# omid-arhami/topolow

Hardware: AMD Instinct MI355X
Metric: relaxation iterations/sec (NxN pairs) (higher is better)
Workload: dtype f32

## Files before the change

topolow_amd/csrc/relax_kernels.h:

```cpp
#pragma once

#include <hip/hip_runtime.h>
#include <type_traits>
#include "relax_common.h"

namespace topolow {

constexpr int kThreads = 256;
constexpr int kWaves = kThreads / 64;

template <int THREADS_, int RPW_, int CHUNK_, int PRIO_ = 0, int MINWAVES_ = 1>
struct StageCfg {
  static constexpr int MINWAVES = MINWAVES_;
  static constexpr int PRIO = PRIO_;
  static constexpr int THREADS = THREADS_;
  static constexpr int WAVES = THREADS_ / 64;
  static constexpr int RPW = RPW_;
  static constexpr int ROWS = WAVES * RPW_;
  static constexpr int CHUNK = CHUNK_;
};

template <typename real> struct Math;
template <> struct Math<float> {
  static __device__ __forceinline__ float sqrt(float x) { return __builtin_amdgcn_sqrtf(x); }
  static __device__ __forceinline__ float rcp(float x) { return __builtin_amdgcn_rcpf(x); }
  static constexpr float far() { return kFarF32; }
};
template <> struct Math<double> {
#ifdef TOPOLOW_F64_IEEE
  static __device__ __forceinline__ double sqrt(double x) { return ::sqrt(x); }
  static __device__ __forceinline__ double rcp(double x) { return 1.0 / x; }
#else
  static __device__ __forceinline__ double sqrt(double x) {
    const double y0 = __builtin_amdgcn_rsq(x);
    double g = x * y0, h = 0.5 * y0;
    const double e1 = fma(-h, g, 0.5);
    g = fma(g, e1, g);
    h = fma(h, e1, h);
    g = fma(fma(-g, g, x), h, g);
    return x > 0.0 ? g : 0.0;
  }
  static __device__ __forceinline__ double rcp(double x) {
    double y = __builtin_amdgcn_rcp(x);
    y = fma(fma(-x, y, 1.0), y, y);
    return fma(fma(-x, y, 1.0), y, y);
  }
#endif
  static constexpr double far() { return kFarF64; }
};

__device__ __forceinline__ float uniform(float v) {
  return __builtin_bit_cast(float, __builtin_amdgcn_readfirstlane(__builtin_bit_cast(int, v)));
}
__device__ __forceinline__ double uniform(double v) {
  const long long b = __builtin_bit_cast(long long, v);
  const int lo = __builtin_amdgcn_readfirstlane((int)(b & 0xffffffffll));
  const int hi = __builtin_amdgcn_readfirstlane((int)(b >> 32));
  return __builtin_bit_cast(double, ((long long)hi << 32) | (unsigned int)lo);
}

template <typename real>
__device__ __forceinline__ real wave_sum(real v) {
#pragma unroll
  for (int m = 32; m >= 1; m >>= 1) v += __shfl_xor(v, m, 64);
  return v;
}

__device__ __forceinline__ float wave_sum_dpp(float v) {
  auto dpp = [](float x, auto ctrl, auto row_mask) {
    return __builtin_bit_cast(float, __builtin_amdgcn_update_dpp(0, __builtin_bit_cast(int, x), decltype(ctrl)::value,
                                                                 decltype(row_mask)::value, 0xf, true));
  };
  using std::integral_constant;
  v += dpp(v, integral_constant<int, 0xB1>{}, integral_constant<int, 0xf>{});
  v += dpp(v, integral_constant<int, 0x4E>{}, integral_constant<int, 0xf>{});
  v += dpp(v, integral_constant<int, 0x141>{}, integral_constant<int, 0xf>{});
  v += dpp(v, integral_constant<int, 0x140>{}, integral_constant<int, 0xf>{});
  v += dpp(v, integral_constant<int, 0x142>{}, integral_constant<int, 0xa>{});
  v += dpp(v, integral_constant<int, 0x143>{}, integral_constant<int, 0xc>{});
  return __builtin_bit_cast(float, __builtin_amdgcn_readlane(__builtin_bit_cast(int, v), 63));
}

typedef __amdgpu_buffer_rsrc_t row_rsrc_t;
__device__ __forceinline__ row_rsrc_t make_row_rsrc(const uint32_t* block, int row_in_block, int ld) {
  const uint32_t* row = block + enc_index(row_in_block, 0, ld);
  return __builtin_amdgcn_make_buffer_rsrc(const_cast<uint32_t*>(row),  0,
                                           enc_row_span_bytes(row_in_block, ld), 0x00020000);
}
__device__ __forceinline__ uint4 load_words(row_rsrc_t rsrc, int byte_off) {
  typedef unsigned int u32x4 __attribute__((ext_vector_type(4)));
  const u32x4 v = __builtin_amdgcn_raw_buffer_load_b128(rsrc, byte_off, 0, 0);
  return make_uint4(v.x, v.y, v.z, v.w);
}

template <int DIM, typename real, int THREADS, int CHUNK>
__device__ __forceinline__ void stage_points(const real* __restrict__ pos, int cb, int cw,
                                             real* lds_pos, int tid) {
  constexpr int kMaxVec = (CHUNK * DIM * (int)sizeof(real) / 16 + THREADS - 1) / THREADS;
  const uint4* src = reinterpret_cast<const uint4*>(pos + (size_t)cb * DIM);
  uint4* dst = reinterpret_cast<uint4*>(lds_pos);
  const int nvec = cw * DIM * (int)sizeof(real) / 16;
  uint4 tmp[kMaxVec];
#pragma unroll
  for (int v = 0; v < kMaxVec; ++v) {
    const int q = tid + v * THREADS;
    tmp[v] = src[q < nvec ? q : 0];
  }
#pragma unroll
  for (int v = 0; v < kMaxVec; ++v) {
    const int q = tid + v * THREADS;
    if (q < nvec) dst[q] = tmp[v];
  }
}

template <int DIM, typename real>
__device__ __forceinline__ void load_points(const real* lds_pos, int c4, real (&pc)[4][DIM]) {
  constexpr int kPer16 = 16 / (int)sizeof(real);
  constexpr int kVec = 4 * DIM / kPer16;
  const uint4* src = reinterpret_cast<const uint4*>(lds_pos + (size_t)c4 * DIM);
#pragma unroll
  for (int v = 0; v < kVec; ++v) {
    const uint4 u = src[v];
    if constexpr (sizeof(real) == 4) {
      pc[(4 * v + 0) / DIM][(4 * v + 0) % DIM] = __builtin_bit_cast(float, u.x);
      pc[(4 * v + 1) / DIM][(4 * v + 1) % DIM] = __builtin_bit_cast(float, u.y);
      pc[(4 * v + 2) / DIM][(4 * v + 2) % DIM] = __builtin_bit_cast(float, u.z);
      pc[(4 * v + 3) / DIM][(4 * v + 3) % DIM] = __builtin_bit_cast(float, u.w);
    } else {
      pc[(2 * v + 0) / DIM][(2 * v + 0) % DIM] =
          __builtin_bit_cast(double, ((unsigned long long)u.y << 32) | u.x);
      pc[(2 * v + 1) / DIM][(2 * v + 1) % DIM] =
          __builtin_bit_cast(double, ((unsigned long long)u.w << 32) | u.z);
    }
  }
}

template <int DIM, typename real, bool THR, bool ERR = false, bool CNT = false>
__device__ __forceinline__ void pair_accum(const real (&pc)[DIM], const real (&pi)[DIM],
                                           uint32_t w, real ks, real cg, real (&acc)[DIM],
                                           float* err = nullptr, unsigned* cnt_wave = nullptr) {
  real dx[DIM];
  real s = 0;
#pragma unroll
  for (int d = 0; d < DIM; ++d) {
    dx[d] = pc[d] - pi[d];
    s = fma(dx[d], dx[d], s);
  }
  const real r = Math<real>::sqrt(s);
  const real inv = Math<real>::rcp(r + (real)0.01);
  const real t = (real)bits_f32(THR ? (w & ~kCodeMask) : w);
  bool spring;
  if constexpr (THR) {
    const uint32_t code = w & kCodeMask;
    spring = (code == 0u) | ((code == 1u) & (r < t)) | ((code == 2u) & (r > t));
  } else {
// ... 528 lines not shown
              pair_error_rows2<DIM, false>(pc[3], pi2, w4[t][0].w, w4[t][1].w, err, cnt_wave);
            }
          }
        }
        if (lane == 0) cnt += cnt_wave;
        err_d += (double)err;
        err = 0.0f;
        continue;
      }
    }
#pragma unroll
    for (int t = 0; t < kGroups; ++t) {
      const int c4 = lane * 4 + t * 256;
      if (c4 >= cw) continue;
      const int col = cb + c4;
      real pc[4][DIM];
      load_points<DIM, real>(lds_pos, c4, pc);
#pragma unroll
      for (int r = 0; r < RPW; ++r) {
        const int i = rows[r];
        bool take[4];
#pragma unroll
        for (int q = 0; q < 4; ++q) {
          const int c = col + q;
          if (PARITY) {
            const bool even = ((i + c) & 1) == 0;
            take[q] = (i != 0x7fffffff) & ((even & (c > i)) | (!even & (c < i)));
          } else {
            take[q] = c > i;
          }
        }
        if (thr) {
          pair_error<DIM, real, true>(pc[0], pi[r], w4[t][r].x, take[0], err, cnt);
          pair_error<DIM, real, true>(pc[1], pi[r], w4[t][r].y, take[1], err, cnt);
          pair_error<DIM, real, true>(pc[2], pi[r], w4[t][r].z, take[2], err, cnt);
          pair_error<DIM, real, true>(pc[3], pi[r], w4[t][r].w, take[3], err, cnt);
        } else {
          pair_error<DIM, real, false>(pc[0], pi[r], w4[t][r].x, take[0], err, cnt);
          pair_error<DIM, real, false>(pc[1], pi[r], w4[t][r].y, take[1], err, cnt);
          pair_error<DIM, real, false>(pc[2], pi[r], w4[t][r].z, take[2], err, cnt);
          pair_error<DIM, real, false>(pc[3], pi[r], w4[t][r].w, take[3], err, cnt);
        }
      }
    }
    err_d += (double)err;
    err = 0.0f;
  }

  double s = wave_sum<double>(err_d);
  unsigned long long c64 = cnt;
#pragma unroll
  for (int m = 32; m >= 1; m >>= 1) c64 += __shfl_xor(c64, m, 64);
  if (lane == 0) { sh_s[wave] = s; sh_c[wave] = c64; }
  __syncthreads();
  if (tid == 0) {
    double ts = 0.0;
    unsigned long long tc = 0;
    for (int w = 0; w < CFG::WAVES; ++w) { ts += sh_s[w]; tc += sh_c[w]; }
    part_sum[part] = ts;
    part_cnt[part] = tc;
  }
}

template <int DIM, typename real, typename tgt_t>
__global__ __launch_bounds__(kThreads) void edge_error_kernel(
    const real* __restrict__ pos, const int* __restrict__ ei, const int* __restrict__ ej,
    const tgt_t* __restrict__ et, const int8_t* __restrict__ ec, long long n_edges,
    double* __restrict__ part_sum, unsigned long long* __restrict__ part_cnt,
    const RunState* st) {
  if (st != nullptr && st->stopped) return;
  double s = 0.0;
  unsigned long long cnt = 0;
  for (long long e = (long long)blockIdx.x * kThreads + threadIdx.x; e < n_edges;
       e += (long long)gridDim.x * kThreads) {
    const int a = ei[e], b = ej[e];
    double q = 0.0;
#pragma unroll
    for (int d = 0; d < DIM; ++d) {
      const double diff = (double)pos[(size_t)b * DIM + d] - (double)pos[(size_t)a * DIM + d];
      q = fma(diff, diff, q);
    }
    const double r = ::sqrt(q);
    const double t = (double)et[e];
    const int c = ec[e];
    const bool contributes = (c == 0) || (c == 1 && r < t) || (c == -1 && r > t);
    if (contributes) { s += fabs(t - r); ++cnt; }
  }
  __shared__ double sh_s[kWaves];
  __shared__ unsigned long long sh_c[kWaves];
  s = wave_sum<double>(s);
#pragma unroll
  for (int m = 32; m >= 1; m >>= 1) cnt += __shfl_xor(cnt, m, 64);
  const int lane = threadIdx.x & 63, wave = threadIdx.x >> 6;
  if (lane == 0) { sh_s[wave] = s; sh_c[wave] = cnt; }
  __syncthreads();
  if (threadIdx.x == 0) {
    double ts = 0.0;
    unsigned long long tc = 0;
    for (int w = 0; w < kWaves; ++w) { ts += sh_s[w]; tc += sh_c[w]; }
    part_sum[blockIdx.x] = ts;
    part_cnt[blockIdx.x] = tc;
  }
}

__global__ __launch_bounds__(1024) void reduce_push_kernel(
    const double* __restrict__ part_sum, const unsigned long long* __restrict__ part_cnt, int n_parts,
    double* const* __restrict__ dst_sum, unsigned long long* const* __restrict__ dst_cnt, int n_dst,
    int slot, const RunState* st) {
  if (st != nullptr && st->stopped) return;
  __shared__ double sh_s[1024];
  __shared__ unsigned long long sh_c[1024];
  double s = 0.0;
  unsigned long long c = 0;
  for (int p = threadIdx.x; p < n_parts; p += 1024) { s += part_sum[p]; c += part_cnt[p]; }
  sh_s[threadIdx.x] = s;
  sh_c[threadIdx.x] = c;
  __syncthreads();
  for (int half = 512; half >= 1; half >>= 1) {
    if (threadIdx.x < half) {
      sh_s[threadIdx.x] += sh_s[threadIdx.x + half];
      sh_c[threadIdx.x] += sh_c[threadIdx.x + half];
    }
    __syncthreads();
  }
  if ((int)threadIdx.x < n_dst) {
    dst_sum[threadIdx.x][slot] = sh_s[0];
    dst_cnt[threadIdx.x][slot] = sh_c[0];
  }
}

__global__ __launch_bounds__(1024) void reduce_total_kernel(
    const double* __restrict__ part_sum, const unsigned long long* __restrict__ part_cnt, int n_parts,
    double* __restrict__ out2, const RunState* st) {
  if (st != nullptr && st->stopped) { if (threadIdx.x == 0) { out2[0] = 0.0; out2[1] = 0.0; } return; }
  __shared__ double sh_s[1024];
  __shared__ unsigned long long sh_c[1024];
  double s = 0.0;
  unsigned long long c = 0;
  for (int p = threadIdx.x; p < n_parts; p += 1024) { s += part_sum[p]; c += part_cnt[p]; }
  sh_s[threadIdx.x] = s;
  sh_c[threadIdx.x] = c;
  __syncthreads();
  for (int half = 512; half >= 1; half >>= 1) {
    if (threadIdx.x < half) {
      sh_s[threadIdx.x] += sh_s[threadIdx.x + half];
      sh_c[threadIdx.x] += sh_c[threadIdx.x + half];
    }
    __syncthreads();
  }
  if (threadIdx.x == 0) { out2[0] = sh_s[0]; out2[1] = (double)sh_c[0]; }
}

constexpr int kCtlThreads = 1024;

template <int THREADS, typename real>
__device__ __forceinline__ void controller_step(
    RunState* st, RunState* mailbox, const double* __restrict__ part_sum,
    const unsigned long long* __restrict__ part_cnt, int n_parts, const real* __restrict__ pos,
    real* __restrict__ best_pos, long long n_values, int iter1, double k_after,
    double* __restrict__ trace, int trace_cap, const double* __restrict__ total2) {
  static_assert(THREADS >= 64 && THREADS <= kCtlThreads && kCtlThreads % THREADS == 0 && (THREADS & (THREADS - 1)) == 0,
                "controller_step: a power-of-two workgroup of at most kCtlThreads threads");
  constexpr int V = kCtlThreads / THREADS;
  if (st->stopped) return;
  __shared__ double sh_s[THREADS];
  __shared__ unsigned long long sh_c[THREADS];
  __shared__ int sh_action;
  double s[V];
  unsigned long long c[V];
#pragma unroll
  for (int j = 0; j < V; ++j) {
    s[j] = 0.0;
    c[j] = 0;
    if (total2 == nullptr)
      for (int p = threadIdx.x + j * THREADS; p < n_parts; p += kCtlThreads) { s[j] += part_sum[p]; c[j] += part_cnt[p]; }
  }
  if (total2 != nullptr && threadIdx.x == 0) { s[0] = total2[0]; c[0] = (unsigned long long)total2[1]; }
#pragma unroll
  for (int h = V / 2; h >= 1; h >>= 1) {
#pragma unroll
    for (int j = 0; j < h; ++j) { s[j] += s[j + h]; c[j] += c[j + h]; }
  }
  sh_s[threadIdx.x] = s[0];
  sh_c[threadIdx.x] = c[0];
  __syncthreads();
  for (int half = THREADS / 2; half >= 1; half >>= 1) {
    if (threadIdx.x < half) {
      sh_s[threadIdx.x] += sh_s[threadIdx.x + half];
      sh_c[threadIdx.x] += sh_c[threadIdx.x + half];
    }
    __syncthreads();
  }
  if (threadIdx.x == 0) {
    const double err = sh_c[0] > 0 ? sh_s[0] / (double)sh_c[0] : 0.0;
    const int action = st->ctl.observe(err, iter1, k_after);
    st->last_mae = err;
    if (trace != nullptr && st->n_checks < trace_cap) {
      trace[3 * st->n_checks + 0] = (double)iter1;
      trace[3 * st->n_checks + 1] = err;
      trace[3 * st->n_checks + 2] = k_after;
    }
    st->n_checks += 1;
    st->iter_base = iter1;
    st->k_base = k_after;
    if (action & 1) { st->stopped = 1; st->converged = 1; }
    sh_action = action;
  }
  __syncthreads();
  if (sh_action & 2) {
    const long long bytes = n_values * (long long)sizeof(real);
    const long long n16 = bytes / 16;
    const uint4* src = reinterpret_cast<const uint4*>(pos);
    uint4* dst = reinterpret_cast<uint4*>(best_pos);
    for (long long q = threadIdx.x; q < n16; q += THREADS) dst[q] = src[q];
    for (long long q = n16 * 16 / (long long)sizeof(real) + threadIdx.x; q < n_values; q += THREADS)
      best_pos[q] = pos[q];
  }
  __syncthreads();
  if (threadIdx.x == 0 && mailbox != nullptr) {
    *mailbox = *st;
    __threadfence_system();
  }
}

template <typename real>
__global__ __launch_bounds__(kCtlThreads) void controller_kernel(
    RunState* st, RunState* mailbox, const double* __restrict__ part_sum,
    const unsigned long long* __restrict__ part_cnt, int n_parts, const real* __restrict__ pos,
    real* __restrict__ best_pos, long long n_values, int iter1, double k_after,
    double* __restrict__ trace, int trace_cap, const double* __restrict__ total2) {
  controller_step<kCtlThreads, real>(st, mailbox, part_sum, part_cnt, n_parts, pos, best_pos, n_values, iter1, k_after,
                                     trace, trace_cap, total2);
}

__global__ __launch_bounds__(kThreads) void encode_dense_kernel(
    const double* __restrict__ D, const int* __restrict__ T, int n, int row_begin, int row_end,
    int ld, uint32_t* __restrict__ out, const int* __restrict__ perm, float* __restrict__ dout) {
  const int c = blockIdx.y * kThreads + threadIdx.x;
  const int i = row_begin + blockIdx.x;
  if (c >= ld || i >= row_end) return;
  uint32_t w = kInfWord;
  float dl = 0.0f;
  if (c < n && c != i) {
    const int oi = perm ? perm[i] : i, oc = perm ? perm[c] : c;
    const int lo = oi < oc ? oi : oc, hi = oi < oc ? oc : oi;
    const size_t cell = (size_t)lo + (size_t)hi * n;
    w = encode_target(D[cell], T[cell]);
    dl = encode_delta(D[cell], w);
  }
  out[enc_index(i - row_begin, c, ld)] = w;
  if (dout != nullptr) dout[enc_index(i - row_begin, c, ld)] = dl;
}

TL_HD inline uint64_t cell_fingerprint(int lo, int hi, uint32_t word) {
  return mix64(((uint64_t)(uint32_t)lo << 32) ^ (uint64_t)(uint32_t)hi ^ ((uint64_t)word * 0x9e3779b97f4a7c15ull));
}
TL_HD inline bool dense_takes(int i, int c, bool parity) {
  if (!parity) return c > i;
  const bool even = ((i + c) & 1) == 0;
  return (even & (c > i)) | (!even & (c < i));
}

__global__ __launch_bounds__(kThreads) void upper_fingerprint_kernel(
    const uint32_t* __restrict__ enc, int n, int row_begin, int row_end, int ld, int parity,
    unsigned long long* __restrict__ out ) {
  const int i = row_begin + blockIdx.x;
  if (i >= row_end) return;
  unsigned long long fp = 0, cnt = 0;
  for (int c = threadIdx.x; c < n; c += kThreads) {
    if (c == i || !dense_takes(i, c, parity != 0)) continue;
    const uint32_t w = enc[enc_index(i - row_begin, c, ld)];
    if (w == kInfWord) continue;
    fp += cell_fingerprint(i < c ? i : c, i < c ? c : i, w);
    ++cnt;
  }
#pragma unroll
  for (int m = 32; m >= 1; m >>= 1) {
    fp += __shfl_xor(fp, m, 64);
    cnt += __shfl_xor(cnt, m, 64);
  }
  if ((threadIdx.x & 63) == 0) {
    atomicAdd(&out[0], fp);
    atomicAdd(&out[1], cnt);
  }
}

__global__ __launch_bounds__(kThreads) void row_flags_kernel(const uint32_t* __restrict__ enc,
                                                             int rows, int ld,
                                                             unsigned char* __restrict__ flags,
                                                             unsigned long long* __restrict__ measured) {
  const int i = blockIdx.x;
  if (i >= rows) return;
  int any = 0;
  unsigned cnt = 0;
  for (int c = threadIdx.x; c < ld; c += kThreads) {
    const uint32_t w = enc[enc_index(i, c, ld)];
    const uint32_t code = w & kCodeMask;
    any |= (code == 1u) | ((code == 2u) & (w != kInfWord));
    cnt += w != kInfWord ? 1u : 0u;
  }
  any = __syncthreads_or(any);
#pragma unroll
  for (int m = 32; m >= 1; m >>= 1) cnt += __shfl_xor(cnt, m, 64);
  if ((threadIdx.x & 63) == 0 && cnt != 0) atomicAdd(measured, (unsigned long long)cnt);
  if (threadIdx.x == 0) flags[i] = any ? 1 : 0;
}

__global__ __launch_bounds__(kThreads) void fill_unmeasured_kernel(
    int n, int row_begin, int row_end, int ld, uint32_t* __restrict__ out, float* __restrict__ dout) {
  const int c = blockIdx.y * kThreads + threadIdx.x;
  const int i = row_begin + blockIdx.x;
  if (c >= ld || i >= row_end) return;
  out[enc_index(i - row_begin, c, ld)] = kInfWord;
  if (dout != nullptr) dout[enc_index(i - row_begin, c, ld)] = 0.0f;
}

__global__ __launch_bounds__(kThreads) void scatter_edges_kernel(
    const int* __restrict__ ei, const int* __restrict__ ej, const double* __restrict__ ed,
    const int* __restrict__ ec, long long n_edges, int n, int row_begin, int row_end, int ld,
    uint32_t* __restrict__ out, const int* __restrict__ inv, float* __restrict__ dout) {
  const long long e = (long long)blockIdx.x * kThreads + threadIdx.x;
  if (e >= n_edges) return;
  int a = ei[e], b = ej[e];
  if (a == b || a < 0 || b < 0 || a >= n || b >= n) return;
  if (inv != nullptr) { a = inv[a]; b = inv[b]; }
  const uint32_t w = encode_target(ed[e], ec[e]);
  if (a >= row_begin && a < row_end) out[enc_index(a - row_begin, b, ld)] = w;
  if (b >= row_begin && b < row_end) out[enc_index(b - row_begin, a, ld)] = w;
  if (dout != nullptr) {
    const float dl = encode_delta(ed[e], w);
    if (a >= row_begin && a < row_end) dout[enc_index(a - row_begin, b, ld)] = dl;
    if (b >= row_begin && b < row_end) dout[enc_index(b - row_begin, a, ld)] = dl;
  }
}

__global__ __launch_bounds__(kThreads) void pdist_kernel(const double* __restrict__ pos, int n,
                                                         int dim, int row0, int rows,
                                                         double* __restrict__ out) {
  const int j = blockIdx.y * kThreads + threadIdx.x;
  const int r = blockIdx.x;
  if (j >= n || r >= rows) return;
  const int i = row0 + r;
  double s = 0.0;
  for (int d = 0; d < dim; ++d) {
    const double dev = pos[(size_t)i * dim + d] - pos[(size_t)j * dim + d];
    s += dev * dev;
  }
  out[(size_t)r * n + j] = ::sqrt(s);
}

}
```

topolow_amd/csrc/relax_symm.h:

```cpp
#pragma once

#include <hip/hip_runtime.h>
#include <algorithm>
#include <type_traits>
#include <vector>
#include "relax_common.h"
#include "relax_kernels.h"

namespace topolow {

#ifndef TOPOLOW_SYM_MINW
#define TOPOLOW_SYM_MINW 2
#endif
constexpr int kSymRows = 64;
constexpr int kSymCols = 32;
constexpr int kSymTileWords = kSymRows * kSymCols;
constexpr int kSymWaves = 4;

template <int DIM> struct SymRec { static constexpr int W = (DIM + 2 + 3) & ~3; };

struct SymUnit {
  int tile_row;
  int j0, j1;
  int tile0;
// ... 323 lines not shown
      request(J, 1, wb);
      u32x4 rn0 = {0, 0, 0, 0}, rn1 = {0, 0, 0, 0};
      rn0 = __builtin_amdgcn_raw_buffer_load_b128(rec_rsrc, (Jn * kTileVec + lane) * 16, 0, 0);
      if constexpr (kTileVec > 64) rn1 = __builtin_amdgcn_raw_buffer_load_b128(rec_rsrc, (Jn * kTileVec + lane + 64) * 16, 0, 0);
      __builtin_amdgcn_sched_barrier(0);

      const bool diag = J < 2 * R + 2;
      float fq[4][W];
#pragma unroll
      for (int q = 0; q < W; ++q) fq[0][q] = f_first[q];
      auto half = [&](auto hc, const u32x4 (&wc)[4]) {
        constexpr int h = decltype(hc)::value;
        symf2 cacc2[2][DIM];
#pragma unroll
        for (int c = 0; c < 2; ++c) {
          if (2 * h + c + 1 < 4) {
            read_rec(J, 2 * h + c + 1, fq[2 * h + c + 1]);
            __builtin_amdgcn_sched_barrier(0);
          }
          const float (&f)[W] = fq[2 * h + c];
          float pc[DIM];
#pragma unroll
          for (int d = 0; d < DIM; ++d) pc[d] = f[d];
          const float ksc = f[DIM], cgc = f[DIM + 1];
#pragma unroll
          for (int p = 0; p < 4; ++p) {
            const uint32_t w0 = c == 0 ? wc[p].x : wc[p].z, w1 = c == 0 ? wc[p].y : wc[p].w;
            if (p == 0)
              sym_pair<DIM, ANYTHR, ERR, ANYTHR, true>(pc, ksc, cgc, pi2[p], ks2[p], cg2[p], w0, w1, racc2[p], cacc2[c], err2, cnt_wave);
            else
              sym_pair<DIM, ANYTHR, ERR, ANYTHR, false>(pc, ksc, cgc, pi2[p], ks2[p], cg2[p], w0, w1, racc2[p], cacc2[c], err2, cnt_wave);
          }
        }
        float first[DIM], second[DIM];
#pragma unroll
        for (int d = 0; d < DIM; ++d) {
          first[d] = cacc2[0][d].x + cacc2[0][d].y;
          second[d] = cacc2[1][d].x + cacc2[1][d].y;
        }
        sym_col_reduce<DIM>(first, second);
        const int off0 = col_off + ((J * kSymCols) * DIM + h * 2 * DIM) * 4;
#pragma unroll
        for (int q = 0; q < DIM; q += 4) {
          if (q + 4 <= DIM) {
            const u32x4 pk = {__builtin_bit_cast(uint32_t, first[q]), __builtin_bit_cast(uint32_t, first[q + 1]),
                              __builtin_bit_cast(uint32_t, first[q + 2]), __builtin_bit_cast(uint32_t, first[q + 3])};
            __builtin_amdgcn_raw_buffer_store_b128(pk, col_rsrc, off0 + q * 4, 0, 0);
          } else {
#pragma unroll
            for (int t = q; t < DIM; ++t)
              __builtin_amdgcn_raw_buffer_store_b32(__builtin_bit_cast(uint32_t, first[t]), col_rsrc, off0 + t * 4, 0, 0);
          }
        }
      };
      half(std::integral_constant<int, 0>{}, wa);
      request(Jn, 0, wa);
      __builtin_amdgcn_sched_barrier(0);
      half(std::integral_constant<int, 1>{}, wb);
      if constexpr (ERR) {
        const float es = err2.x + err2.y;
        err_unit += diag ? es : 2.0f * es;
        cnt_unit2 += diag ? cnt_wave : 2u * cnt_wave;
        err2 = (symf2){0.0f, 0.0f};
        cnt_wave = 0;
      }
      __builtin_amdgcn_sched_barrier(0);
      if (lane < kTileVec) lds[wave][(J + 1) & 1][lds_slot(lane)] = make_uint4(rn0.x, rn0.y, rn0.z, rn0.w);
      if constexpr (kTileVec > 64) if (lane + 64 < kTileVec) lds[wave][(J + 1) & 1][lds_slot(lane + 64)] = make_uint4(rn1.x, rn1.y, rn1.z, rn1.w);
      read_rec(J + 1, 0, f_first);
    }
#pragma unroll
    for (int p = 0; p < 4; ++p)
#pragma unroll
      for (int d = 0; d < DIM; ++d) {
        symf2 v = racc2[p][d];
        v.x += __shfl_xor(v.x, 8, 64);  v.y += __shfl_xor(v.y, 8, 64);
        v.x += __shfl_xor(v.x, 16, 64); v.y += __shfl_xor(v.y, 16, 64);
        v.x += __shfl_xor(v.x, 32, 64); v.y += __shfl_xor(v.y, 32, 64);
        racc2[p][d] = v;
      }
    if (b == 0) {
      float* dst = rowpart + ((size_t)slot * kSymRows + 8 * a) * DIM;
#pragma unroll
      for (int p = 0; p < 4; ++p)
#pragma unroll
        for (int d = 0; d < DIM; ++d) {
          dst[(2 * p) * DIM + d] = racc2[p][d].x;
          dst[(2 * p + 1) * DIM + d] = racc2[p][d].y;
        }
    }
    if constexpr (ERR) {
      double s = (double)err_unit;
#pragma unroll
      for (int m = 32; m >= 1; m >>= 1) s += __shfl_xor(s, m, 64);
      if constexpr (ANYTHR) {
#pragma unroll
        for (int m = 32; m >= 1; m >>= 1) cnt_unit2 += __shfl_xor(cnt_unit2, m, 64);
      }
      if (lane == 0) {
        part_sum[slot] = s;
        part_cnt[slot] = ANYTHR ? (unsigned long long)cnt_unit2 : (slot == 0 ? fixed_cnt : 0ull);
      }
    }
  }
#ifdef TOPOLOW_SYM_STAMPS
  if (lane == 0 && g_sym_stamps != nullptr) {
    g_sym_stamps[4 * gw] = __builtin_amdgcn_s_memtime() - stamp_c0;
    g_sym_stamps[4 * gw + 1] = stamp_r0;
    g_sym_stamps[4 * gw + 2] = __builtin_amdgcn_s_memrealtime();
    unsigned hw_id, xcc_id;
    asm volatile("s_getreg_b32 %0, hwreg(HW_REG_HW_ID)" : "=s"(hw_id));
    asm volatile("s_getreg_b32 %0, hwreg(HW_REG_XCC_ID)" : "=s"(xcc_id));
    g_sym_stamps[4 * gw + 3] = ((unsigned long long)xcc_id << 32) | hw_id;
  }
#endif
}

template <int DIM, typename real> struct SymReal;
template <int DIM> struct SymReal<DIM, float> {
  static constexpr int W = SymRec<DIM>::W;
  __device__ static float ks(double k, float g) { return (float)(2.0 * k) / (4.0f * g + (float)k); }
  __device__ static float cg(double c_rep, float g) { return (float)(0.5 * c_rep) / g; }
  __device__ static float far(int) { return kFarF32; }
};

struct SymApplyCheck {
  const double* part_sum = nullptr;
  const unsigned long long* part_cnt = nullptr;
  int n_parts = 0;
  const void* pos = nullptr;
  void* best = nullptr;
  long long n_values = 0;
  int iter1 = 0;
  double k_after = 0.0;
  double* trace = nullptr;
  int trace_cap = 0;
  RunState* mailbox = nullptr;
};

#ifndef TL_APPLY_PARTS
#define TL_APPLY_PARTS 16
#endif
constexpr int kSymApplyParts = TL_APPLY_PARTS;
template <int DIM, typename real>
__global__ __launch_bounds__(32 * kSymApplyParts) void symm_apply_kernel(
    const real* __restrict__ rec, real* __restrict__ rec_next, real* __restrict__ pos_out, const float* __restrict__ gplus,
    const real* __restrict__ rowpart, const real* __restrict__ colpart, const int2* __restrict__ row_units, int n,
    int npad, double k_next, double c_rep, int iter1, RunState* st, int rr_stages = 0, int rr_stage = 0,
    SymApplyCheck chk = SymApplyCheck{}) {
  const bool check_wg = (int)blockIdx.x * kSymCols >= npad;
  const int R = check_wg ? 0 : blockIdx.x >> 1;
  const int2 ru = row_units[R];
  int stopped = st->stopped;
  asm("" : "+s"(stopped) : "s"(ru.x), "s"(ru.y), "s"(rec), "s"(rowpart), "s"(colpart), "s"(n), "s"(npad), "s"(rr_stages), "s"(rr_stage),
      "s"(rec_next), "s"(pos_out), "s"(gplus), "s"(k_next), "s"(c_rep));
  if (stopped) return;
  if (check_wg) {
    if (chk.part_sum != nullptr)
      controller_step<32 * kSymApplyParts, real>(st, chk.mailbox, chk.part_sum, chk.part_cnt, chk.n_parts,
                                                 (const real*)chk.pos, (real*)chk.best, chk.n_values, chk.iter1,
                                                 chk.k_after, chk.trace, chk.trace_cap, nullptr);
    return;
  }
  using T = SymReal<DIM, real>;
  constexpr int W = T::W;
  constexpr int kWavesA = kSymApplyParts / 2;
  __shared__ real red[kWavesA][kSymCols][DIM];
  const int part = threadIdx.x >> 5, pt = threadIdx.x & 31;
  const int i = blockIdx.x * kSymCols + pt;
  real acc[DIM];
#pragma unroll
  for (int d = 0; d < DIM; ++d) acc[d] = 0;
  int rp0 = 0, rp1 = R;
  if (rr_stages > 0) sym_rr_above(npad / kSymRows, rr_stages, rr_stage, R, rp0, rp1);
  for (int Rp = rp0 + part; Rp < rp1; Rp += kSymApplyParts) {
    const real* src = colpart + ((size_t)Rp * npad + i) * DIM;
#pragma unroll
    for (int d = 0; d < DIM; ++d) acc[d] += src[d];
  }
  const int row_in_tile = i - R * kSymRows;
  for (int q = part; q < ru.y; q += kSymApplyParts) {
    const real* src = rowpart + ((size_t)(ru.x + q) * kSymRows + row_in_tile) * DIM;
#pragma unroll
    for (int d = 0; d < DIM; ++d) acc[d] -= src[d];
  }
#pragma unroll
  for (int d = 0; d < DIM; ++d) {
    if constexpr (std::is_same<real, float>::value) acc[d] += __shfl_xor(acc[d], 32, 64);
    else acc[d] += T::lane_xor(acc[d], 32);
  }
  const int wave = threadIdx.x >> 6;
  if ((threadIdx.x & 32) == 0) {
#pragma unroll
    for (int d = 0; d < DIM; ++d) red[wave][pt][d] = acc[d];
  }
  __syncthreads();
  if (part == 0 && i < n) {
    bool finite = true;
    real out[DIM];
#pragma unroll
    for (int d = 0; d < DIM; ++d) {
      real t = red[0][pt][d];
#pragma unroll
      for (int p = 1; p < kWavesA; ++p) t += red[p][pt][d];
      out[d] = rec[(size_t)i * W + d] + t;
      finite = finite && isfinite(out[d]);
      pos_out[(size_t)i * DIM + d] = out[d];
      rec_next[(size_t)i * W + d] = out[d];
    }
    const real g = (real)gplus[i];
    rec_next[(size_t)i * W + DIM] = T::ks(k_next, g);
    rec_next[(size_t)i * W + DIM + 1] = T::cg(c_rep, g);
    if (!finite) atomicMin(&st->first_nonfinite, iter1);
  }
}

template <int DIM, typename real>
__global__ __launch_bounds__(256) void symm_records_kernel(const real* __restrict__ pos, const float* __restrict__ gplus,
                                                          real* __restrict__ rec, int n, int npad, double k, double c_rep) {
  using T = SymReal<DIM, real>;
  constexpr int W = T::W;
  const int i = blockIdx.x * blockDim.x + threadIdx.x;
  if (i >= npad) return;
  real* r = rec + (size_t)i * W;
  if (i < n) {
#pragma unroll
    for (int d = 0; d < DIM; ++d) r[d] = pos[(size_t)i * DIM + d];
    const real g = (real)gplus[i];
    r[DIM] = T::ks(k, g);
    r[DIM + 1] = T::cg(c_rep, g);
  } else {
#pragma unroll
    for (int d = 0; d < DIM; ++d) r[d] = T::far(d);
    r[DIM] = 0;
    r[DIM + 1] = 0;
  }
#pragma unroll
  for (int d = DIM + 2; d < W; ++d) r[d] = 0;
}

__global__ __launch_bounds__(256) void symm_tiles_kernel(const uint32_t* const* __restrict__ src, const int* __restrict__ row0,
                                                        int n_src, int ld, uint32_t* __restrict__ tenc, int TC,
                                                        long long t_first, uint32_t fill) {
  const long long t = t_first + blockIdx.x;
  int R = 0;
  {
    const double b = (double)TC + 1.0;
    const double disc = b * b - 4.0 * (double)t;
    R = (int)((b - sqrt(disc > 0.0 ? disc : 0.0)) * 0.5);
    while (R > 0 && (long long)R * TC - (long long)R * (R - 1) > t) --R;
    while ((long long)(R + 1) * TC - (long long)(R + 1) * R <= t) ++R;
  }
  const int J = 2 * R + (int)(t - ((long long)R * TC - (long long)R * (R - 1)));
  uint32_t* dst = tenc + (size_t)blockIdx.x * kSymTileWords;
  const int rows = row0[n_src];
#pragma unroll
  for (int q = 0; q < kSymTileWords / 256; ++q) {
    const int cell = threadIdx.x + q * 256;
    const int r = cell >> 5, c = cell & 31;
    const int row = R * kSymRows + r, col = J * kSymCols + c;
    uint32_t w = fill;
    if (row < rows && col < ld) {
      int blk = 0;
      while (blk + 1 < n_src && row >= row0[blk + 1]) ++blk;
      w = src[blk][enc_index(row - row0[blk], col, ld)];
    }
    const int a = r >> 3, p = (r & 7) >> 1, e = r & 1, b = c >> 2, h = (c & 3) >> 1, f = c & 1;
    dst[(((4 * h + p) * 64) + a + 8 * b) * 4 + 2 * (f ^ (a & 1)) + e] = w;
  }
}


template <int DIM>
__global__ __launch_bounds__(32 * 32) void symm_partial_kernel(
    const float* __restrict__ rowpart, const float* __restrict__ colpart, const int2* __restrict__ row_units, int r_first,
    int r_last, int n, int npad, float* const* __restrict__ inbox, const int* __restrict__ own0, int n_own, int slot,
    const RunState* st) {
  if (st != nullptr && st->stopped) return;
  __shared__ float red[32][kSymCols][DIM];
  const int R = blockIdx.x >> 1;
  const int part = threadIdx.x >> 5, pt = threadIdx.x & 31;
  const int i = blockIdx.x * kSymCols + pt;
  float acc[DIM];
#pragma unroll
  for (int d = 0; d < DIM; ++d) acc[d] = 0.0f;
  const int r_stop = R < r_last + 1 ? R : r_last + 1;
  for (int Rp = r_first + part; Rp < r_stop; Rp += 32) {
    const float* src = colpart + ((size_t)(Rp - r_first) * npad + i) * DIM;
#pragma unroll
    for (int d = 0; d < DIM; ++d) acc[d] += src[d];
  }
  if (R >= r_first && R <= r_last) {
    const int2 ru = row_units[R - r_first];
    const int row_in_tile = i - R * kSymRows;
    for (int q = part; q < ru.y; q += 32) {
      const float* src = rowpart + ((size_t)(ru.x + q) * kSymRows + row_in_tile) * DIM;
#pragma unroll
      for (int d = 0; d < DIM; ++d) acc[d] -= src[d];
    }
  }
#pragma unroll
  for (int d = 0; d < DIM; ++d) red[part][pt][d] = acc[d];
  __syncthreads();
  if (part == 0 && i < n) {
    int q = 0;
    while (q + 1 < n_own && i >= own0[q + 1]) ++q;
    float* dst = inbox[q] + ((size_t)slot * npad + i) * DIM;
#pragma unroll
    for (int d = 0; d < DIM; ++d) {
      float t = red[0][pt][d];
#pragma unroll
      for (int p = 1; p < 32; ++p) t += red[p][pt][d];
      dst[d] = t;
    }
// ... 30 lines not shown
```

Measured before the change: 18100.

## Hoist controller loads ahead of stop check and batch partial-sum reads

The controller step now issues its first partial-sum loads before the stopped-flag check, so their latency overlaps that check. It reads the controller state with wide buffer loads, batches the remaining partial loads, and finishes the reduction with a wave shuffle instead of LDS steps down to one thread. The best-position copy is batched eight vectors per thread and runs after the mailbox write. This shortens the serial latency chain of the convergence check. The cost is added complexity and bounds-checked buffer loads that may run even when the run has already stopped.

```diff
diff --git a/topolow_amd/csrc/relax_kernels.h b/topolow_amd/csrc/relax_kernels.h
--- a/topolow_amd/csrc/relax_kernels.h
+++ b/topolow_amd/csrc/relax_kernels.h
@@ -1,6 +1,7 @@
 #pragma once
 
 #include <hip/hip_runtime.h>
+#include <cstddef>
 #include <type_traits>
 #include "relax_common.h"
 
@@ -835,28 +836,96 @@
 }
 
 constexpr int kCtlThreads = 1024;
-
+constexpr int kCtlCopyBatch = 8;
+
+struct CtlFirst {
+  double s;
+  unsigned long long c;
+};
+__device__ __forceinline__ CtlFirst controller_first(const double* part_sum, const unsigned long long* part_cnt, int n_parts) {
+  typedef unsigned int u32x2 __attribute__((ext_vector_type(2)));
+  const __amdgpu_buffer_rsrc_t rs = __builtin_amdgcn_make_buffer_rsrc(const_cast<double*>(part_sum), 0, n_parts * 8, 0x00020000);
+  const __amdgpu_buffer_rsrc_t rc = __builtin_amdgcn_make_buffer_rsrc(const_cast<unsigned long long*>(part_cnt), 0, n_parts * 8, 0x00020000);
+  const u32x2 vs = __builtin_amdgcn_raw_buffer_load_b64(rs, (int)threadIdx.x * 8, 0, 0);
+  const u32x2 vc = __builtin_amdgcn_raw_buffer_load_b64(rc, (int)threadIdx.x * 8, 0, 0);
+  CtlFirst f;
+  f.s = __builtin_bit_cast(double, vs);
+  f.c = __builtin_bit_cast(unsigned long long, vc);
+  return f;
+}
+
+struct CtlView {
+  Controller ctl;
+  int n_checks;
+};
+__device__ __forceinline__ CtlView controller_view(const RunState* st) {
+  static_assert(sizeof(Controller) == 40 && offsetof(RunState, ctl) == 0, "controller_view: the controller as 16 + 16 + 8 bytes");
+  typedef unsigned int u32x2 __attribute__((ext_vector_type(2)));
+  typedef unsigned int u32x4 __attribute__((ext_vector_type(4)));
+  struct Words { uint32_t w[10]; };
+  const __amdgpu_buffer_rsrc_t rsrc = __builtin_amdgcn_make_buffer_rsrc(const_cast<RunState*>(st), 0, (int)sizeof(RunState), 0x00020000);
+  const int off = threadIdx.x == 0 ? 0 : 0x40000000;
+  const u32x4 a = __builtin_amdgcn_raw_buffer_load_b128(rsrc, off, 0, 0);
+  const u32x4 b = __builtin_amdgcn_raw_buffer_load_b128(rsrc, off + 16, 0, 0);
+  const u32x2 c = __builtin_amdgcn_raw_buffer_load_b64(rsrc, off + 32, 0, 0);
+  const uint32_t n = __builtin_amdgcn_raw_buffer_load_b32(rsrc, off + (int)offsetof(RunState, n_checks), 0, 0);
+  const Words w = {{a.x, a.y, a.z, a.w, b.x, b.y, b.z, b.w, c.x, c.y}};
+  CtlView v;
+  v.ctl = __builtin_bit_cast(Controller, w);
+  v.n_checks = (int)n;
+  return v;
+}
+
+constexpr int kCtlPartBatch = 4;
 template <int THREADS, typename real>
 __device__ __forceinline__ void controller_step(
     RunState* st, RunState* mailbox, const double* __restrict__ part_sum,
     const unsigned long long* __restrict__ part_cnt, int n_parts, const real* __restrict__ pos,
     real* __restrict__ best_pos, long long n_values, int iter1, double k_after,
-    double* __restrict__ trace, int trace_cap, const double* __restrict__ total2) {
-  static_assert(THREADS >= 64 && THREADS <= kCtlThreads && kCtlThreads % THREADS == 0 && (THREADS & (THREADS - 1)) == 0,
+    double* __restrict__ trace, int trace_cap, const double* __restrict__ total2, CtlFirst first) {
+  static_assert(THREADS >= 128 && THREADS <= kCtlThreads && kCtlThreads % THREADS == 0 && (THREADS & (THREADS - 1)) == 0,
                 "controller_step: a power-of-two workgroup of at most kCtlThreads threads");
   constexpr int V = kCtlThreads / THREADS;
-  if (st->stopped) return;
   __shared__ double sh_s[THREADS];
   __shared__ unsigned long long sh_c[THREADS];
   __shared__ int sh_action;
+  const CtlView view = controller_view(st);
   double s[V];
   unsigned long long c[V];
 #pragma unroll
   for (int j = 0; j < V; ++j) {
     s[j] = 0.0;
     c[j] = 0;
-    if (total2 == nullptr)
-      for (int p = threadIdx.x + j * THREADS; p < n_parts; p += kCtlThreads) { s[j] += part_sum[p]; c[j] += part_cnt[p]; }
+  }
+  if (total2 == nullptr) {
+    const __amdgpu_buffer_rsrc_t rs = __builtin_amdgcn_make_buffer_rsrc(const_cast<double*>(part_sum), 0, n_parts * 8, 0x00020000);
+    const __amdgpu_buffer_rsrc_t rc = __builtin_amdgcn_make_buffer_rsrc(const_cast<unsigned long long*>(part_cnt), 0, n_parts * 8, 0x00020000);
+    auto batch = [&](auto first_here, int m0) {
+      double vs[V][kCtlPartBatch];
+      unsigned long long vc[V][kCtlPartBatch];
+#pragma unroll
+      for (int j = 0; j < V; ++j)
+#pragma unroll
+        for (int k = 0; k < kCtlPartBatch; ++k) {
+          if (decltype(first_here)::value && j == 0 && k == 0) {
+            vs[j][k] = first.s;
+            vc[j][k] = first.c;
+          } else {
+            const int p = (int)threadIdx.x + j * THREADS + (m0 + k) * kCtlThreads;
+            vs[j][k] = __builtin_bit_cast(double, __builtin_amdgcn_raw_buffer_load_b64(rs, p * 8, 0, 0));
+            vc[j][k] = __builtin_bit_cast(unsigned long long, __builtin_amdgcn_raw_buffer_load_b64(rc, p * 8, 0, 0));
+          }
+        }
+#pragma unroll
+      for (int j = 0; j < V; ++j)
+#pragma unroll
+        for (int k = 0; k < kCtlPartBatch; ++k) {
+          const int p = (int)threadIdx.x + j * THREADS + (m0 + k) * kCtlThreads;
+          if (p < n_parts) { s[j] += vs[j][k]; c[j] += vc[j][k]; }
+        }
+    };
+    batch(std::true_type{}, 0);
+    for (int m0 = kCtlPartBatch; m0 * kCtlThreads < n_parts; m0 += kCtlPartBatch) batch(std::false_type{}, m0);
   }
   if (total2 != nullptr && threadIdx.x == 0) { s[0] = total2[0]; c[0] = (unsigned long long)total2[1]; }
 #pragma unroll
@@ -867,43 +936,81 @@
   sh_s[threadIdx.x] = s[0];
   sh_c[threadIdx.x] = c[0];
   __syncthreads();
-  for (int half = THREADS / 2; half >= 1; half >>= 1) {
+  for (int half = THREADS / 2; half >= 128; half >>= 1) {
     if (threadIdx.x < half) {
       sh_s[threadIdx.x] += sh_s[threadIdx.x + half];
       sh_c[threadIdx.x] += sh_c[threadIdx.x + half];
     }
     __syncthreads();
   }
-  if (threadIdx.x == 0) {
-    const double err = sh_c[0] > 0 ? sh_s[0] / (double)sh_c[0] : 0.0;
-    const int action = st->ctl.observe(err, iter1, k_after);
-    st->last_mae = err;
-    if (trace != nullptr && st->n_checks < trace_cap) {
-      trace[3 * st->n_checks + 0] = (double)iter1;
-      trace[3 * st->n_checks + 1] = err;
-      trace[3 * st->n_checks + 2] = k_after;
-    }
-    st->n_checks += 1;
-    st->iter_base = iter1;
-    st->k_base = k_after;
-    if (action & 1) { st->stopped = 1; st->converged = 1; }
-    sh_action = action;
-  }
-  __syncthreads();
-  if (sh_action & 2) {
-    const long long bytes = n_values * (long long)sizeof(real);
-    const long long n16 = bytes / 16;
-    const uint4* src = reinterpret_cast<const uint4*>(pos);
-    uint4* dst = reinterpret_cast<uint4*>(best_pos);
-    for (long long q = threadIdx.x; q < n16; q += THREADS) dst[q] = src[q];
-    for (long long q = n16 * 16 / (long long)sizeof(real) + threadIdx.x; q < n_values; q += THREADS)
-      best_pos[q] = pos[q];
+  if (threadIdx.x < 64) {
+    double ts = sh_s[threadIdx.x] + sh_s[threadIdx.x + 64];
+    unsigned long long tc = sh_c[threadIdx.x] + sh_c[threadIdx.x + 64];
+#pragma unroll
+    for (int half = 32; half >= 1; half >>= 1) {
+      ts += __shfl_down(ts, half, 64);
+      tc += __shfl_down(tc, half, 64);
+    }
+    if (threadIdx.x == 0) {
+      const double err = tc > 0 ? ts / (double)tc : 0.0;
+      Controller ctl = view.ctl;
+      const int action = ctl.observe(err, iter1, k_after);
+      st->ctl = ctl;
+      st->last_mae = err;
+      if (trace != nullptr && view.n_checks < trace_cap) {
+        trace[3 * view.n_checks + 0] = (double)iter1;
+        trace[3 * view.n_checks + 1] = err;
+        trace[3 * view.n_checks + 2] = k_after;
+      }
+      st->n_checks = view.n_checks + 1;
+      st->iter_base = iter1;
+      st->k_base = k_after;
+      if (action & 1) { st->stopped = 1; st->converged = 1; }
+      sh_action = action;
+    }
   }
   __syncthreads();
   if (threadIdx.x == 0 && mailbox != nullptr) {
     *mailbox = *st;
     __threadfence_system();
   }
+  if (sh_action & 2) {
+    const long long bytes = n_values * (long long)sizeof(real);
+    const long long n16 = bytes / 16;
+    typedef unsigned int u32x4 __attribute__((ext_vector_type(4)));
+    const u32x4* src = reinterpret_cast<const u32x4*>(pos);
+    u32x4* dst = reinterpret_cast<u32x4*>(best_pos);
+    static_assert(kCtlCopyBatch == 8, "controller_step: the statement below names the batch's pieces");
+#define TL_CTL_PIN_BATCH(v) \
+  asm volatile("" : "+v"(v[0]), "+v"(v[1]), "+v"(v[2]), "+v"(v[3]), "+v"(v[4]), "+v"(v[5]), "+v"(v[6]), "+v"(v[7]))
+    long long q = threadIdx.x;
+    for (; q + (long long)(kCtlCopyBatch - 1) * THREADS < n16; q += (long long)kCtlCopyBatch * THREADS) {
+      u32x4 v[kCtlCopyBatch];
+#pragma unroll
+      for (int k = 0; k < kCtlCopyBatch; ++k) v[k] = src[q + (long long)k * THREADS];
+      TL_CTL_PIN_BATCH(v);
+#pragma unroll
+      for (int k = 0; k < kCtlCopyBatch; ++k) dst[q + (long long)k * THREADS] = v[k];
+    }
+    if (q < n16) {
+      u32x4 v[kCtlCopyBatch];
+#pragma unroll
+      for (int k = 0; k < kCtlCopyBatch; ++k) {
+        const long long qk = q + (long long)k * THREADS;
+        v[k] = src[qk < n16 ? qk : q];
+      }
+      TL_CTL_PIN_BATCH(v);
+#pragma unroll
+      for (int k = 0; k < kCtlCopyBatch; ++k) {
+        const long long qk = q + (long long)k * THREADS;
+        if (qk < n16) dst[qk] = v[k];
+      }
+    }
+#undef TL_CTL_PIN_BATCH
+    for (long long t = n16 * 16 / (long long)sizeof(real) + threadIdx.x; t < n_values; t += THREADS)
+      best_pos[t] = pos[t];
+  }
+  __syncthreads();
 }
 
 template <typename real>
@@ -912,8 +1019,12 @@
     const unsigned long long* __restrict__ part_cnt, int n_parts, const real* __restrict__ pos,
     real* __restrict__ best_pos, long long n_values, int iter1, double k_after,
     double* __restrict__ trace, int trace_cap, const double* __restrict__ total2) {
+  const CtlFirst first = controller_first(part_sum, part_cnt, total2 == nullptr ? n_parts : 0);
+  int stopped = st->stopped;
+  asm("" : "+s"(stopped) : "v"(first.s), "v"(first.c));
+  if (stopped) return;
   controller_step<kCtlThreads, real>(st, mailbox, part_sum, part_cnt, n_parts, pos, best_pos, n_values, iter1, k_after,
-                                     trace, trace_cap, total2);
+                                     trace, trace_cap, total2, first);
 }
 
 __global__ __launch_bounds__(kThreads) void encode_dense_kernel(
diff --git a/topolow_amd/csrc/relax_symm.h b/topolow_amd/csrc/relax_symm.h
--- a/topolow_amd/csrc/relax_symm.h
+++ b/topolow_amd/csrc/relax_symm.h
@@ -499,14 +499,15 @@
   const int R = check_wg ? 0 : blockIdx.x >> 1;
   const int2 ru = row_units[R];
   int stopped = st->stopped;
+  const CtlFirst chk_first = controller_first(chk.part_sum, chk.part_cnt, check_wg && chk.part_sum != nullptr ? chk.n_parts : 0);
   asm("" : "+s"(stopped) : "s"(ru.x), "s"(ru.y), "s"(rec), "s"(rowpart), "s"(colpart), "s"(n), "s"(npad), "s"(rr_stages), "s"(rr_stage),
-      "s"(rec_next), "s"(pos_out), "s"(gplus), "s"(k_next), "s"(c_rep));
+      "s"(rec_next), "s"(pos_out), "s"(gplus), "s"(k_next), "s"(c_rep), "v"(chk_first.s), "v"(chk_first.c));
   if (stopped) return;
   if (check_wg) {
     if (chk.part_sum != nullptr)
       controller_step<32 * kSymApplyParts, real>(st, chk.mailbox, chk.part_sum, chk.part_cnt, chk.n_parts,
                                                  (const real*)chk.pos, (real*)chk.best, chk.n_values, chk.iter1,
-                                                 chk.k_after, chk.trace, chk.trace_cap, nullptr);
+                                                 chk.k_after, chk.trace, chk.trace_cap, nullptr, chk_first);
     return;
   }
   using T = SymReal<DIM, real>;
```

New measurement: 18110 (median of 2 runs). No clear change (+0.1%).
